# cherubicXN/neat

Hardware: AMD Instinct MI355X
Metric: ray-samples/s (train step) on ABC-neat-a (higher is better)
Workload: dtype bf16; 1 GPU; C2: abc-neat-a networks, 1024 rays x 128 samples per GPU, depth samples given, train step = forward + loss + backward + Adam; rays_per_gpu=1024, samples_per_ray=128, global_rays=1024, parallelism=dp1, weights=synthetic 'rough' (seed 42), launch=hip graph replay, the whole step one launch (forward + loss + backward + Adam)

## Files before the change

neat_amd/csrc/bf16_common.hpp:

```cpp
#pragma once
#include <hip/hip_runtime.h>
#include <stdint.h>

#ifndef NEAT_HALF
#define NEAT_HALF 0
#endif

namespace neat {

struct DevOnce {
  unsigned long long mask = 0;
  static int dev() { int d = 0; if (hipGetDevice(&d) != hipSuccess || d < 0 || d > 63) d = 0; return d; }
  operator bool() const { return ((mask >> dev()) & 1ull) != 0; }
  DevOnce& operator=(bool v) { if (v) mask |= 1ull << dev(); else mask &= ~(1ull << dev()); return *this; }
};
#define NEAT_TRY(expr) do { hipError_t e_ = (expr); if (e_ != hipSuccess) return e_; } while (0)
template <auto... Kerns> hipError_t lds_limit(int bytes) {
  static DevOnce done;
  if (done) return hipSuccess;
  hipError_t e = hipSuccess;
  ((e = e != hipSuccess ? e : hipFuncSetAttribute(reinterpret_cast<const void*>(Kerns), hipFuncAttributeMaxDynamicSharedMemorySize, bytes)), ...);
  if (e == hipSuccess) done = true;
  return e;
}

typedef float f32x16 __attribute__((ext_vector_type(16)));
typedef unsigned short u16;

constexpr int BMH = 128;

typedef float f32x2_t __attribute__((ext_vector_type(2)));
#if NEAT_HALF
typedef _Float16 bf16x8 __attribute__((ext_vector_type(8)));
typedef _Float16 bf16x2_t __attribute__((ext_vector_type(2)));
#define NEAT_MFMA16 __builtin_amdgcn_mfma_f32_32x32x16_f16
__device__ __forceinline__ unsigned pack2(float lo, float hi) {
  f32x2_t v = {lo, hi};
  bf16x2_t r = __builtin_convertvector(v, bf16x2_t);
  return __builtin_bit_cast(unsigned, r);
}
__device__ __forceinline__ u16 f2bf(float f) { return __builtin_bit_cast(u16, (_Float16)f); }
__device__ __forceinline__ float bf2f(u16 h) { return (float)__builtin_bit_cast(_Float16, h); }
__device__ __forceinline__ float bf_lo(unsigned w) { return (float)__builtin_bit_cast(bf16x2_t, w).x; }
__device__ __forceinline__ float bf_hi(unsigned w) { return (float)__builtin_bit_cast(bf16x2_t, w).y; }
#else
typedef __bf16 bf16x8 __attribute__((ext_vector_type(8)));
typedef __bf16 bf16x2_t __attribute__((ext_vector_type(2)));
#define NEAT_MFMA16 __builtin_amdgcn_mfma_f32_32x32x16_bf16
__device__ __forceinline__ unsigned pack2(float lo, float hi) {
  f32x2_t v = {lo, hi};
  bf16x2_t r = __builtin_convertvector(v, bf16x2_t);
  return __builtin_bit_cast(unsigned, r);
}
__device__ __forceinline__ u16 f2bf(float f) { return (u16)(pack2(f, 0.0f) & 0xFFFFu); }
__device__ __forceinline__ float bf2f(u16 h) { return __uint_as_float(((unsigned)h) << 16); }
__device__ __forceinline__ float bf_lo(unsigned w) { return __uint_as_float(w << 16); }
__device__ __forceinline__ float bf_hi(unsigned w) { return __uint_as_float(w & 0xFFFF0000u); }
#endif

typedef short s16x2_t __attribute__((ext_vector_type(2)));
typedef unsigned short u16x2_t __attribute__((ext_vector_type(2)));
__device__ __forceinline__ unsigned pk_relu16(unsigned p) {
  const s16x2_t z = {0, 0};
  return __builtin_bit_cast(unsigned, __builtin_elementwise_max(__builtin_bit_cast(s16x2_t, p), z));
}
__device__ __forceinline__ unsigned pk_nonzero16(unsigned p) {
  unsigned r;
  asm("v_pk_min_u16 %0, %1, %2" : "=v"(r) : "v"(p), "s"(0x00010001u));
  return r;
}
typedef float pk2f_t __attribute__((ext_vector_type(2)));
__device__ __forceinline__ pk2f_t pk_add_f32(pk2f_t a, pk2f_t b) {
  pk2f_t r;
  asm("v_pk_add_f32 %0, %1, %2" : "=v"(r) : "v"(a), "v"(b));
  return r;
}
__device__ __forceinline__ void relu_mask_push(unsigned& m, unsigned relu_pair) { m = (m << 1) | pk_nonzero16(relu_pair); }
__device__ __forceinline__ unsigned relu_mask_word(unsigned m) { return m << 8; }
__device__ __forceinline__ unsigned relu_mask_apply(unsigned& m, unsigned pair) {
  const s16x2_t sh = {15, 15};
  const unsigned keep = __builtin_bit_cast(unsigned, __builtin_bit_cast(s16x2_t, m) >> sh);
  m <<= 1;
  return pair & keep;
}

__device__ __forceinline__ float softplus100_fast(float a) {
  const float u = a * 144.26950408889634f;
  const float y = __builtin_amdgcn_exp2f(-fabsf(u));
  return (fmaxf(u, 0.0f) + __builtin_amdgcn_logf(1.0f + y)) * 0.0069314718055994531f;
}
typedef float v2f_t __attribute__((ext_vector_type(2)));
constexpr float SOFTPLUS_C = 144.26950408889634f;
__device__ __forceinline__ v2f_t softplus100_pk(v2f_t acc, v2f_t bias_scaled) {
  const v2f_t cc = {SOFTPLUS_C, SOFTPLUS_C};
  const v2f_t u = acc * cc + bias_scaled;
  v2f_t y = {__builtin_amdgcn_exp2f(-fabsf(u.x)), __builtin_amdgcn_exp2f(-fabsf(u.y))};
  const v2f_t one = {1.0f, 1.0f};
  y = y + one;
  const v2f_t lg = {__builtin_amdgcn_logf(y.x), __builtin_amdgcn_logf(y.y)};
  const v2f_t m = {fmaxf(u.x, 0.0f), fmaxf(u.y, 0.0f)};
  const v2f_t k = {0.0069314718055994531f, 0.0069314718055994531f};
  return (m + lg) * k;
}
__device__ __forceinline__ float dphi_fast(float h) { return 1.0f - __expf(-100.0f * h); }

struct FusedArgs {
  const float* x_fm; int P, ldp;
  const uint4* Wp[9]; int KS[9]; const float* bias[9];
  int save, values_only;
  u16* h[9];
  float* E;
  u16* feat; float* sdfraw;
  const uint4* Wlo[9]; u16* hlo[9]; u16* featlo;
  float* sdf_out;
  float radius, scale;
  int bias8_rot, bias8_n;
  const int* gate; int gate_value;
};

struct AdjArgs {
  int P, ldp;
  const uint4* Wp[8];
  const u16* h[9];
  u16* u[8];
  const float* w8; const float* rs8;
  float* es; float* e0;
  const uint4* Wlo[8]; const u16* hlo[9];
};

struct HeadX3Args {
  int P, ldp;
  int nvalid;
  const u16* feat; const u16* featlo;
  const float* small; int srows;
  const uint4* Wp[5]; const uint4* Wlo[5];
  const float* bias[5];
  u16* hid[5];
  float* out;
  const u16* smallbf;
  u16* mask[5];
};

struct HeadBwdArgs {
  int P, ldp;
  int nvalid;
  const u16* top;
  const uint4* Wt[5];
  const u16* mask[5];
  u16* ab[4];
  u16* featc;
  int accumulate;
  const float* rho_num; const float* rho_den;
  float* sc; int srows;
};

}
```

neat_amd/csrc/kernels_dw.hpp:

```cpp
#pragma once
#include "kernels_bf16.hpp"

namespace neat {

struct LayerArgsDW {
  LayerArgsWS w;
  const u16* auxA2; int auxA_split;
  int rowsA;
  int P;
  uint4* partial;
  float* pscale;
  float* pbias;
  int ablate;
};

constexpr int DW_MAXSEG = 4;
struct LayerArgsDWSeg { LayerArgsDW l[DW_MAXSEG]; int n; };

constexpr int DW_XLDS = 1024;
constexpr int DW_WG_UINT4 = 8 * 8 * 2 * 64;
#ifndef DW_VALU_PER_MFMA
#define DW_VALU_PER_MFMA 14
#endif

__device__ __forceinline__ unsigned long long dw_uniform64(unsigned long long v) {
  const unsigned lo = __builtin_amdgcn_readfirstlane((unsigned)v), hi = __builtin_amdgcn_readfirstlane((unsigned)(v >> 32));
  return ((unsigned long long)hi << 32) | lo;
}
__device__ __forceinline__ void dw_dma16(unsigned long long sbase, unsigned voff, unsigned lds_dst) {
  unsigned keep;
  asm volatile("s_mov_b32 %0, m0\n\ts_mov_b32 m0, %2\n\ts_nop 0\n\tglobal_load_lds_dwordx4 %1, %3 nt\n\ts_mov_b32 m0, %0"
               : "=&s"(keep) : "v"(voff), "s"(lds_dst), "s"(sbase) : "memory");
}
__device__ __forceinline__ void dw_dma4(unsigned long long sbase, unsigned voff, unsigned lds_dst) {
  unsigned keep;
  asm volatile("s_mov_b32 %0, m0\n\ts_mov_b32 m0, %2\n\ts_nop 0\n\tglobal_load_lds_dword %1, %3\n\ts_mov_b32 m0, %0"
               : "=&s"(keep) : "v"(voff), "s"(lds_dst), "s"(sbase) : "memory");
}

template <int EPI, bool FULL>
__global__ __launch_bounds__(WST, 2) void layer_kernel_wsdw(LayerArgsDWSeg seg) {
  constexpr bool SEG = FULL && EPI != EPI_BWD8;
  typedef WsCfg<EPI, 16> C;
  static_assert(C::NAUX == 2, "tangent / reverse epilogues only");
  constexpr bool TANK = (EPI == EPI_TAN || EPI == EPI_TAN_PF);
  const LayerArgsDW* tab = (const LayerArgsDW*)__builtin_amdgcn_kernarg_segment_ptr();
  const int nlayers = SEG ? seg.n : 1;
  for (int li = 0; li < nlayers; ++li) {
  if (SEG && li > 0) {
    asm volatile("s_waitcnt vmcnt(0)" ::: "memory");
    __syncthreads();
  }
  const LayerArgsDW d = SEG ? tab[li] : seg.l[0];
  const LayerArgsWS& a = d.w;
  extern __shared__ __attribute__((aligned(16))) unsigned char wslds[];
  typedef __attribute__((address_space(3))) void* lds_ptr;
  typedef __attribute__((address_space(3))) v4s16* lds_v4;
  const int lane0 = threadIdx.x & 63;
  const int wave = __builtin_amdgcn_readfirstlane(threadIdx.x >> 6);
  const int t_begin = (int)blockIdx.x, tstride = (int)gridDim.x;
  const int T = (a.ntiles - t_begin + tstride - 1) / tstride;
  const unsigned lds_base = (unsigned)(size_t)(lds_ptr)wslds;
  const unsigned dma_off = (unsigned)(4 * wave) * (WSP * 16);
  constexpr unsigned AUX0 = C::IN_TILE, AUX1 = C::IN_TILE + WS_TILE, EXTRA = C::IN_TILE + WS_TILE * C::NAUX;
  constexpr unsigned AUXA = TANK ? AUX1 : AUX0;
  auto lane_now = [&]() { int l = lane0; asm volatile("" : "+v"(l)); return l; };
  auto dma = [&](const u16* base, int ln, int tile, unsigned dst, int max_oct, const u16* base2, int split) {
    const bool second = 4 * wave >= split;
    const unsigned long long sb = dw_uniform64((unsigned long long)(second ? base2 : base) + (unsigned long long)tile * (WSP * 16));
    const int o0 = second ? 4 * wave - split : 4 * wave;
#pragma unroll
    for (int i = 0; i < 2; ++i) {
      const int opos = 2 * i + (ln >> 5);
      const int oct = min(o0 + opos, second ? 31 : max_oct);
      const unsigned voff = ((unsigned)oct * (unsigned)a.ldp + (unsigned)((ln & 31) ^ (opos << 2))) * 16u;
      dw_dma16(sb, voff, __builtin_amdgcn_readfirstlane(dst + i * (2 * WSP * 16)));
    }
  };
  auto issue = [&](int tau) {
    const unsigned stage = lds_base + (unsigned)(tau % C::NS) * C::STAGE;
    const unsigned slot = stage + dma_off;
    const int tile = t_begin + tau * tstride;
    const int ln = lane_now();
    dma(a.in, ln, tile, slot, a.in_octs - 1, a.in2, a.split_oct);
    dma(a.aux0, ln, tile, slot + AUX0, 31, TANK ? nullptr : d.auxA2, TANK ? (1 << 30) : d.auxA_split);
    dma(a.aux1, ln, tile, slot + AUX1, 31, TANK ? d.auxA2 : nullptr, TANK ? d.auxA_split : (1 << 30));
    if (C::HAS_S) dw_dma4(dw_uniform64((unsigned long long)(a.srow + (size_t)tile * WSP)), (unsigned)(ln & 31) * 4u, __builtin_amdgcn_readfirstlane(stage + EXTRA + wave * 256));
    if (C::HAS_PF) dw_dma16(dw_uniform64((unsigned long long)(a.padfill + (size_t)tile * WSP * 8)), (unsigned)(ln & 31) * 16u, __builtin_amdgcn_readfirstlane(stage + EXTRA));
  };
#pragma unroll
  for (int t = 0; t < C::NS - 1; ++t)
    if (t < T) issue(t);

  const bool live = FULL || wave * 32 < a.N;
  uint4 wreg[16];
#pragma unroll
  for (int ks = 0; ks < 16; ++ks) wreg[ks] = live ? a.Wp[((size_t)wave * a.kstride + ks) * 64 + lane0] : make_uint4(0u, 0u, 0u, 0u);
  float* w8 = reinterpret_cast<float*>(wslds + C::LDS);
  if (EPI == EPI_BWD8 && threadIdx.x < 256) w8[threadIdx.x] = (int)threadIdx.x < a.N ? a.wrow[threadIdx.x] * a.wrow_scale[0] : 0.0f;
  const int Npad = (a.N + 7) & ~7;

  f32x16 dacc[8];
#pragma unroll
  for (int j = 0; j < 8; ++j)
#pragma unroll
    for (int r = 0; r < 16; ++r) dacc[j][r] = 0.0f;
  float bsum[2] = {0.0f, 0.0f};
  const int wr = 64 * (wave >> 1), wc = 128 * (wave & 1);
  const bool BIAS = d.pbias != nullptr && wc == 0;

  for (int tau = 0; tau < T; ++tau) {
    const int ahead = min(C::NS - 2, T - 1 - tau);
    ws_wait_barrier(ahead * C::G);
    if (tau + C::NS - 1 < T) issue(tau + C::NS - 1);
    const unsigned char* slot = wslds + (tau % C::NS) * C::STAGE;
    const int tile = t_begin + tau * tstride;
    const int ln = lane_now();
    const unsigned hi5 = (unsigned)(ln >> 5), l31 = (unsigned)(ln & 31);
    const unsigned G = (unsigned)(ln >> 4), li = (unsigned)(ln & 15);
    const unsigned ol = 2 * (G & 1) + ((li >> 1) & 1);
    const unsigned tro0 = ol * 512 + (((2 * (G >> 1)) ^ ol) * 4 + (li >> 2)) * 16 + (li & 1) * 8;
    const unsigned tro1 = ol * 512 + (((2 * (G >> 1) + 1) ^ ol) * 4 + (li >> 2)) * 16 + (li & 1) * 8;
    const bool tail = (tile + 1) * WSP > d.P;
    const unsigned char* abase = (TANK ? slot + AUX1 : slot) + (wr >> 5) * 2048;
    const unsigned char* bbase = (TANK ? slot : slot + AUX0) + (wc >> 5) * 2048;
    auto frag = [&](const unsigned char* base, int s2) {
      const v4s16 lo = __builtin_amdgcn_ds_read_tr16_b64_v4i16((lds_v4)(base + tro0 + s2 * 256));
      const v4s16 hi = __builtin_amdgcn_ds_read_tr16_b64_v4i16((lds_v4)(base + tro1 + s2 * 256));
      return make_uint4(((const unsigned*)&lo)[0], ((const unsigned*)&lo)[1], ((const unsigned*)&hi)[0], ((const unsigned*)&hi)[1]);
    };
    auto load_frags = [&](int s2, uint4 (&av)[2], uint4 (&bv)[4]) {
#pragma unroll
      for (int i = 0; i < 2; ++i) av[i] = frag(abase + i * 2048, s2);
#pragma unroll
      for (int j = 0; j < 4; ++j) bv[j] = frag(bbase + j * 2048, s2);
    };
    auto mask_frags = [&](int s2, uint4 (&av)[2], uint4 (&bv)[4], bool points) {
      const int arow = wr + (int)(16 * (G & 1) + li);
      const unsigned amask0 = arow < d.rowsA ? 0xFFFFFFFFu : 0u, amask1 = arow + 32 < d.rowsA ? 0xFFFFFFFFu : 0u;
      av[0].x &= amask0; av[0].y &= amask0; av[0].z &= amask0; av[0].w &= amask0;
      av[1].x &= amask1; av[1].y &= amask1; av[1].z &= amask1; av[1].w &= amask1;
      if (!points) return;
      auto mask4 = [&](uint4& v) {
        const int p0 = tile * WSP + 16 * s2 + 8 * (int)(G >> 1);
        unsigned w4[4] = {v.x, v.y, v.z, v.w};
#pragma unroll
        for (int e = 0; e < 4; ++e) {
          const bool k0 = p0 + 2 * e < d.P, k1 = p0 + 2 * e + 1 < d.P;
          w4[e] = (k0 ? (w4[e] & 0x0000FFFFu) : 0u) | (k1 ? (w4[e] & 0xFFFF0000u) : 0u);
        }
        v = make_uint4(w4[0], w4[1], w4[2], w4[3]);
      };
#pragma unroll
      for (int i = 0; i < 2; ++i) mask4(av[i]);
#pragma unroll
      for (int j = 0; j < 4; ++j) mask4(bv[j]);
    };
    auto dw_mma = [&](const uint4 (&av)[2], const uint4 (&bv)[4], bool mfma = true) {
      if (!TANK && BIAS) {
#pragma unroll
        for (int i = 0; i < 2; ++i) {
          const unsigned w4[4] = {av[i].x, av[i].y, av[i].z, av[i].w};
          float t = 0.0f;
#pragma unroll
          for (int e = 0; e < 4; ++e) t += bf_lo(w4[e]) + bf_hi(w4[e]);
          bsum[i] += t;
        }
      }
      if (!mfma) return;
#pragma unroll
      for (int i = 0; i < 2; ++i)
#pragma unroll
        for (int j = 0; j < 4; ++j)
          dacc[i * 4 + j] = NEAT_MFMA16(*reinterpret_cast<const bf16x8*>(&av[i]), *reinterpret_cast<const bf16x8*>(&bv[j]), dacc[i * 4 + j], 0, 0, 0);
    };
    f32x16 acc;
    auto chain = [&]() {
#pragma unroll
      for (int r = 0; r < 16; ++r) acc[r] = 0.0f;
      const unsigned bfrag_e = (hi5 * WSP + (l31 ^ (hi5 << 2))) * 16;
      const unsigned bfrag_o = (hi5 * WSP + (l31 ^ ((2 + hi5) << 2))) * 16;
#pragma unroll
      for (int ks = 0; ks < 16; ++ks) {
        const uint4 bv = *reinterpret_cast<const uint4*>(slot + ((ks & 1) ? bfrag_o : bfrag_e) + ks * (2 * WSP * 16));
        acc = NEAT_MFMA16(*reinterpret_cast<const bf16x8*>(&wreg[ks]), *reinterpret_cast<const bf16x8*>(&bv), acc, 0, 0, 0);
      }
    };
    const int p = tile * WSP + (int)l31;
    auto epi_half = [&](int j, bool fullrows, const uint4* fa = nullptr, const uint4* fb = nullptr) {
      float sp = 0.0f;
      if (C::HAS_S) sp = *reinterpret_cast<const float*>(slot + EXTRA + wave * 256 + l31 * 4);
// ... 195 lines not shown
```

neat_amd/csrc/kernels_heads.hpp:

```cpp
#pragma once
#include "bf16_common.hpp"
#include "fused_launch.hpp"

namespace neat {

struct HC {
  static constexpr int BP = HC_BATCH, THREADS = 512;
  static constexpr int XPL = 32 * BP * 16;
  static constexpr int SPL = 8 * BP * 16;
  static constexpr int XA = 0, XB = XPL, S = 2 * XPL;
  static constexpr int BIAS = S + SPL;
  static constexpr int BIAS_FLOATS = 4 * 256 + 8;
  static constexpr int LDS = BIAS + BIAS_FLOATS * 4;
  static constexpr int KSTEP = 2 * BP * 16;
};

#ifndef NEAT_HC_RING
#define NEAT_HC_RING 3
#endif
#ifndef NEAT_HC_ABLATE
#define NEAT_HC_ABLATE 0
#endif

#ifndef NEAT_HC_NT_FWD
#define NEAT_HC_NT_FWD 1
#endif
#ifndef NEAT_HC_NT_BWD
#define NEAT_HC_NT_BWD 0
#endif
template <bool NT = false>
__device__ __forceinline__ void hc_store8(void* p, uint2 v) {
  typedef unsigned long long u64_t;
  if (NT) __builtin_nontemporal_store(__builtin_bit_cast(u64_t, v), reinterpret_cast<u64_t*>(p));
  else *reinterpret_cast<uint2*>(p) = v;
}
#ifndef NEAT_HC_WIDE
#define NEAT_HC_WIDE 1
#endif
__device__ __forceinline__ uint4 hc_octet(uint2 prev, uint2 cur) {
  typedef unsigned v2u_t __attribute__((ext_vector_type(2)));
  const v2u_t s0 = __builtin_amdgcn_permlane32_swap(prev.x, cur.x, false, false);
  const v2u_t s1 = __builtin_amdgcn_permlane32_swap(prev.y, cur.y, false, false);
  return make_uint4(s0.x, s1.x, s0.y, s1.y);
}
template <bool NT = false>
__device__ __forceinline__ void hc_store16(void* p, uint4 v) {
  typedef unsigned v4u_t __attribute__((ext_vector_type(4)));
  const v4u_t w = {v.x, v.y, v.z, v.w};
  if (NT) __builtin_nontemporal_store(w, reinterpret_cast<v4u_t*>(p));
  else *reinterpret_cast<v4u_t*>(p) = w;
}
#ifndef NEAT_HC_TIMING
#define NEAT_HC_TIMING 0
#endif
#if NEAT_HC_TIMING
#define HC_STAMP(i) do { if (blockIdx.x == 0 && it < 3) { __builtin_amdgcn_s_waitcnt(0); stamp[i] = __builtin_readcyclecounter(); } } while (0)
#else
#define HC_STAMP(i) do { } while (0)
#endif

__device__ __forceinline__ uint4 hc_ldg(const void* base, unsigned off) {
  return *reinterpret_cast<const uint4*>(reinterpret_cast<const unsigned char*>(base) + off);
}
#ifndef NEAT_HC_NT_IN
#define NEAT_HC_NT_IN 0
#endif
__device__ __forceinline__ uint4 hc_ldg_in(const void* base, unsigned off) {
  typedef unsigned v4u_t __attribute__((ext_vector_type(4)));
  if (NEAT_HC_NT_IN) {
    const v4u_t v = __builtin_nontemporal_load(reinterpret_cast<const v4u_t*>(reinterpret_cast<const unsigned char*>(base) + off));
    return make_uint4(v.x, v.y, v.z, v.w);
  }
  return hc_ldg(base, off);
}

template <int KS, bool ZERO, bool ROLL, int NKS, int WN, class Epi>
__device__ __forceinline__ void hc_stage(const unsigned char* fr, uint4 (&w)[WN], f32x16& acc, const void* wn, unsigned woff, Epi&& epi) {
  constexpr int RING = NEAT_HC_RING;
  uint4 b[KS];
#pragma unroll
  for (int i = 0; i < RING && i < KS; ++i) b[i] = *reinterpret_cast<const uint4*>(fr + i * HC::KSTEP);
  if (ROLL) {
#pragma unroll
    for (int ks = KS; ks < NKS; ++ks) w[ks] = hc_ldg(wn, woff + ks * 1024);
  }
  if (ZERO) {
#pragma unroll
    for (int r = 0; r < 16; ++r) acc[r] = 0.0f;
  }
#pragma unroll
  for (int ks = 0; ks < KS; ++ks) {
    if (ks + RING < KS) b[ks + RING] = *reinterpret_cast<const uint4*>(fr + (ks + RING) * HC::KSTEP);
    if (!(NEAT_HC_ABLATE & 2))
      acc = NEAT_MFMA16(*reinterpret_cast<const bf16x8*>(&w[ks]), *reinterpret_cast<const bf16x8*>(&b[ks]), acc, 0, 0, 0);
    else acc[0] += __uint_as_float(w[ks].x ^ b[ks].x);
    if (ROLL && ks < NKS) w[ks] = hc_ldg(wn, woff + ks * 1024);
    if (!(NEAT_HC_ABLATE & 1)) {
#pragma unroll
      for (int e = ks * (16 / KS); e < (ks + 1) * (16 / KS); ++e) epi(e);
    }
    __builtin_amdgcn_sched_barrier(0);
  }
}
template <class Epi> __device__ __forceinline__ void hc_drain(Epi&& epi) {
#pragma unroll
  for (int e = 0; e < 16; ++e) { epi(e); if ((e & 3) == 3) __builtin_amdgcn_sched_barrier(0); }
}

#ifndef NEAT_HC_STAGGER
#define NEAT_HC_STAGGER 0
#endif
struct HcWork {
  int rounds, tail0, grid, nvp;
  __device__ __forceinline__ HcWork(int nvalid_pairs, int g) : grid(g), nvp(nvalid_pairs) {
    rounds = (nvalid_pairs / 2) / g;
    tail0 = rounds * g * 2;
  }
  __device__ __forceinline__ int batch(int it, int bid, int& pair0) const {
    if (NEAT_HC_STAGGER && (bid & 1) && rounds > 0) {
      if (it == 0) { pair0 = 2 * bid; return 1; }
      if (it == rounds) { pair0 = 2 * bid + 1; return 1; }
      if (it > rounds) --it;
    }
    if (it < rounds) { pair0 = 2 * (it * grid + bid); return 2; }
    pair0 = tail0 + (it - rounds) * grid + bid;
    return pair0 < nvp ? 1 : 0;
  }
};

template <int HEAD, bool SAVE>
__global__ __launch_bounds__(512, 2) void head_chain_kernel(HeadX3Args a, int npairs) {
  typedef HC C;
  constexpr int BP = C::BP, NOUT = HEAD ? 6 : 3;
  extern __shared__ __attribute__((aligned(16))) unsigned char hclds[];
  float* biasl = reinterpret_cast<float*>(hclds + C::BIAS);
  const int tid = threadIdx.x, lane = tid & 63, hi = lane >> 5;
  const int wave = __builtin_amdgcn_readfirstlane(tid >> 6);
  for (int idx = tid; idx < 4 * 256; idx += C::THREADS) {
    const int l = idx >> 8, n = idx & 255;
    float v = 0.0f;
#pragma unroll
    for (int k = 0; k < 4; ++k) if (l == k) v = a.bias[k][n];
    biasl[idx] = v;
  }
  if (tid < 8) biasl[4 * 256 + tid] = tid < NOUT ? a.bias[4][tid] : 0.0f;
  for (int idx = tid; idx < C::SPL / 16; idx += C::THREADS) reinterpret_cast<uint4*>(hclds + C::S)[idx] = make_uint4(0u, 0u, 0u, 0u);

  const int nvp = npairs < a.nvalid ? npairs : a.nvalid;
  for (int pair = nvp + blockIdx.x; pair < npairs; pair += gridDim.x) {
    const unsigned p0 = (unsigned)pair * 64u;
    if (SAVE) {
#pragma unroll
      for (int l = 1; l <= 4; ++l) {
#pragma unroll
        for (int i = 0; i < 4; ++i) {
          const int idx = tid + i * C::THREADS, oct = idx >> 6, pp = idx & 63;
          *reinterpret_cast<uint4*>(reinterpret_cast<char*>(a.hid[l]) + ((unsigned)oct * (unsigned)a.ldp + p0 + pp) * 16u) = make_uint4(0u, 0u, 0u, 0u);
        }
        if (tid < 256) reinterpret_cast<uint4*>(reinterpret_cast<char*>(a.mask[l]) + (size_t)pair * 4096)[tid] = make_uint4(0u, 0u, 0u, 0u);
      }
    }
    for (int idx = tid; idx < NOUT * 64; idx += C::THREADS) a.out[(size_t)(idx >> 6) * a.ldp + p0 + (idx & 63)] = 0.0f;
  }

  uint4 w[20], ow[2];
  auto w_off = [&](int KS) -> unsigned {
    unsigned v = (unsigned)((wave * KS) * 64 + lane) * 16u;
    asm volatile("" : "+v"(v));
    return v;
  };
  {
    const unsigned o0 = w_off(20);
#pragma unroll
    for (int ks = 0; ks < 20; ++ks) w[ks] = hc_ldg(a.Wp[0], o0 + ks * 1024);
    unsigned so = (unsigned)(((2 * wave) * 64 + lane) * 16);
    asm volatile("" : "+v"(so));
#pragma unroll
    for (int j = 0; j < 2; ++j) ow[j] = hc_ldg(a.Wp[4], so + j * 1024);
  }
  const unsigned char* frag[3];
  unsigned char* quad[2];
  const unsigned char* biasp;
  {
    const unsigned fo = (unsigned)(hi * BP + (lane & 31)) * 16u, qo = (unsigned)((4 * wave) * BP + (lane & 31)) * 16u + 8u * hi;
    unsigned b0 = C::XA + fo, b1 = C::XB + fo, b2 = C::S + fo, q0 = C::XA + qo, q1 = C::XB + qo, bb = C::BIAS + (unsigned)(32 * wave + 4 * hi) * 4u;
    asm volatile("" : "+v"(b0), "+v"(b1), "+v"(b2), "+v"(q0), "+v"(q1), "+v"(bb));
    frag[0] = hclds + b0; frag[1] = hclds + b1; frag[2] = hclds + b2;
    quad[0] = hclds + q0; quad[1] = hclds + q1; biasp = hclds + bb;
  }
  __syncthreads();

  const HcWork work(nvp, gridDim.x);
  for (int it = 0;; ++it) {
    int pair0;
    const int np = work.batch(it, blockIdx.x, pair0);
    if (np == 0) break;
    const int nt = 2 * np, npts = 64 * np;
#if NEAT_HC_TIMING
    unsigned long long stamp[8];
#endif
    HC_STAMP(0);
    const unsigned p0 = (unsigned)pair0 * 64u;
    unsigned ldp16 = (unsigned)a.ldp * 16u;
    asm volatile("" : "+s"(ldp16));
    const unsigned gquad = ((unsigned)(4 * wave) * (unsigned)a.ldp + p0 + (unsigned)(lane & 31)) * 16u + 8u * hi;
    const unsigned goct = ((unsigned)(4 * wave + hi) * (unsigned)a.ldp + p0 + (unsigned)(lane & 31)) * 16u;
    const unsigned mlane = (((p0 >> 5) * 8u + (unsigned)wave) * 64u + (unsigned)lane) * 4u;
    int tb = tid;
    asm volatile("" : "+v"(tb));
    {
#pragma unroll
      for (int i = 0; i < 8; ++i) {
        const int idx = tb + i * C::THREADS, oct = idx >> 7, pp = idx & 127;
        if (pp < npts) reinterpret_cast<uint4*>(hclds + C::XA)[oct * BP + pp] = hc_ldg_in(a.feat, ((unsigned)oct * (unsigned)a.ldp + p0 + pp) * 16u);
      }
      const int so = tb >> 7, sp = tb & 127;
      for (int o = so; o * 8 < a.srows; o += 4)
        if (sp < npts) reinterpret_cast<uint4*>(hclds + C::S)[o * BP + sp] = hc_ldg_in(a.smallbf, ((unsigned)o * (unsigned)a.ldp + p0 + sp) * 16u);
    }
    __syncthreads();
    HC_STAMP(1);

    f32x16 acc[2];
    unsigned pboff = 0;
    unsigned char* plq = quad[0];
    unsigned pg = 0;
    u16* phout = nullptr; u16* pmout = nullptr; unsigned pmoff = 0;
    float4 bqv = make_float4(0.f, 0.f, 0.f, 0.f);
    unsigned ph[2]; float keep = 0.0f; unsigned mbits = 0;
    uint2 vprev = make_uint2(0u, 0u);
    unsigned pgw = 0;
    auto epi_elem = [&](const f32x16& ap, int e) {
      if (NEAT_HC_ABLATE & 64) {
        keep += ap[e];
        if (e == 15 && keep == 12345.0f) *reinterpret_cast<float*>(plq) = keep;
        return;
      }
      const int q = e >> 2, j = e & 3;
      if (j == 0 && !(NEAT_HC_ABLATE & 32)) bqv = *reinterpret_cast<const float4*>(biasp + pboff + q * 32);
      if ((j & 1) == 0) return;
      const v2f_t av = {ap[e - 1], ap[e]};
      const v2f_t bv = (j == 1) ? v2f_t{bqv.x, bqv.y} : v2f_t{bqv.z, bqv.w};
#ifndef NEAT_HC_PK_BIAS
#define NEAT_HC_PK_BIAS 0
#endif
      const v2f_t rv = NEAT_HC_PK_BIAS ? pk_add_f32(av, bv) : v2f_t{av.x + bv.x, av.y + bv.y};
      const unsigned pr = pk_relu16(pack2(rv.x, rv.y));
      ph[j >> 1] = pr;
      if (SAVE && !(NEAT_HC_ABLATE & 8)) relu_mask_push(mbits, pr);
      if (j != 3) return;
      const uint2 vh = make_uint2(ph[0], ph[1]);
      if (!(NEAT_HC_ABLATE & 16)) *reinterpret_cast<uint2*>(plq + q * (BP * 16)) = vh;
      if (SAVE) {
        if (NEAT_HC_WIDE) {
          if (q & 1) hc_store16<NEAT_HC_NT_FWD != 0>(reinterpret_cast<char*>(phout) + (size_t)(q - 1) * ldp16 + pgw, hc_octet(vprev, vh));
          else vprev = vh;
        } else if (!(NEAT_HC_ABLATE & 4)) hc_store8<NEAT_HC_NT_FWD != 0>(reinterpret_cast<char*>(phout) + (size_t)q * ldp16 + pg, vh);
#ifndef NEAT_HC_NT_MASK
#define NEAT_HC_NT_MASK 1
#endif
        if (q == 3 && !(NEAT_HC_ABLATE & 8)) {
          if (NEAT_HC_NT_MASK) __builtin_nontemporal_store(relu_mask_word(mbits), reinterpret_cast<unsigned*>(reinterpret_cast<char*>(pmout) + pmoff));
          else *reinterpret_cast<unsigned*>(reinterpret_cast<char*>(pmout) + pmoff) = relu_mask_word(mbits);
          mbits = 0;
        }
      }
    };
    auto set_pend = [&](int l, int dst, int t) {
      pboff = (unsigned)l * 1024u;
      plq = quad[dst] + t * 512;
      pg = gquad + (unsigned)t * 512u;
      pgw = goct + (unsigned)t * 512u;
      phout = a.hid[l + 1]; pmout = a.mask[l + 1]; pmoff = mlane + (unsigned)t * 2048u;
    };
    auto none = [](int) {};
    auto seed = [&](f32x16& ac, int t) {
#pragma unroll
      for (int r = 0; r < 16; ++r) ac[r] = 0.0f;
#pragma unroll
      for (int ks = 0; ks < 4; ++ks) {
        const uint4 bs = *reinterpret_cast<const uint4*>(frag[2] + t * 512 + ks * C::KSTEP);
        ac = NEAT_MFMA16(*reinterpret_cast<const bf16x8*>(&w[16 + ks]), *reinterpret_cast<const bf16x8*>(&bs), ac, 0, 0, 0);
      }
    };
#define HC_EPI(ACC_) [&](int e) { epi_elem(ACC_, e); }
#define HC_LAYER(LL, SRC_, DST_, WN_, KSN_)                                                                                        \
    for (int pp = 0; pp < np; ++pp) {                                                                                             \
      const int t0 = 2 * pp;                                                                                                      \
      if (LL == 0) seed(acc[0], t0);                                                                                              \
      if (LL == 0 && pp == 0) {                                                                                                   \
        hc_stage<16, false, false, 16>(frag[SRC_] + t0 * 512, w, acc[0], nullptr, 0u, none);                                       \
      } else {                                                                                                                    \
        if (pp == 0) set_pend(LL - 1, SRC_, nt - 1); else set_pend(LL, DST_, t0 - 1);                                              \
        hc_stage<16, LL != 0, false, 16>(frag[SRC_] + t0 * 512, w, acc[0], nullptr, 0u, HC_EPI(acc[1]));                           \
      }                                                                                                                           \
      if (np == 1 && !(NEAT_HC_ABLATE & 128)) __syncthreads();                                                                    \
      if (LL == 0) seed(acc[1], t0 + 1);                                                                                          \
      set_pend(LL, DST_, t0);                                                                                                     \
      if (pp == np - 1) hc_stage<16, LL != 0, true, 16>(frag[SRC_] + (t0 + 1) * 512, w, acc[1], WN_, w_off(KSN_), HC_EPI(acc[0])); \
      else hc_stage<16, LL != 0, false, 16>(frag[SRC_] + (t0 + 1) * 512, w, acc[1], nullptr, 0u, HC_EPI(acc[0]));                  \
      if (!(NEAT_HC_ABLATE & 128)) __syncthreads();                                                                               \
    }
#define HC_LAYER3 HC_LAYER(3, 1, 0, a.Wp[0], 20)
    HC_LAYER(0, 0, 1, a.Wp[1], 16)
    HC_STAMP(2);
    HC_LAYER(1, 1, 0, a.Wp[2], 16)
    HC_STAMP(3);
    HC_LAYER(2, 0, 1, a.Wp[3], 16)
    HC_STAMP(4);
    HC_LAYER3
    set_pend(3, 0, nt - 1);
    hc_drain(HC_EPI(acc[1]));
    __syncthreads();
    HC_STAMP(5);
#undef HC_LAYER3
#undef HC_LAYER
#undef HC_EPI
    {
      float* red = reinterpret_cast<float*>(hclds + C::XB);
      const unsigned char* fr = frag[0] + (unsigned)(2 * wave) * C::KSTEP;
      for (int t = 0; t < nt; ++t) {
        f32x16 accs;
#pragma unroll
        for (int r = 0; r < 16; ++r) accs[r] = 0.0f;
#pragma unroll
        for (int j = 0; j < 2; ++j) {
          const uint4 bh = *reinterpret_cast<const uint4*>(fr + j * C::KSTEP + t * 512);
          accs = NEAT_MFMA16(*reinterpret_cast<const bf16x8*>(&ow[j]), *reinterpret_cast<const bf16x8*>(&bh), accs, 0, 0, 0);
        }
#pragma unroll
        for (int r = 0; r < 4; ++r) red[(wave * 8 + 4 * hi + r) * BP + t * 32 + (lane & 31)] = accs[r];
      }
      __syncthreads();
      int tf = tid;
      asm volatile("" : "+v"(tf));
      for (int idx = tf; idx < NOUT * BP; idx += C::THREADS) {
        const int n = idx >> 7, pp = idx & 127;
        if (pp < npts) {
          float v = biasl[4 * 256 + n];
#pragma unroll
          for (int wv = 0; wv < 8; ++wv) v += red[(wv * 8 + n) * BP + pp];
          if (HEAD == 0) v = 1.0f / (1.0f + __expf(-v));
          a.out[(size_t)n * a.ldp + p0 + pp] = v;
        }
      }
    }
    __syncthreads();
    HC_STAMP(6);
#if NEAT_HC_TIMING
    if (blockIdx.x == 0 && it < 3 && (tid == 0 || tid == 448))
      printf("hc fwd head %d wave %d batch %d (np %d): load %llu lin0 %llu lin1 %llu lin2 %llu lin3 %llu lin4 %llu cycles\n", HEAD, wave, it, np,
             stamp[1] - stamp[0], stamp[2] - stamp[1], stamp[3] - stamp[2], stamp[4] - stamp[3], stamp[5] - stamp[4], stamp[6] - stamp[5]);
#endif
  }
}


__device__ __forceinline__ float hc_cot_scale_of(const float* slot) {
  if (!slot) return 1.0f;
  const float m = *slot;
  if (!(m > 0.0f) || !(m < 3.0e38f)) return 1.0f;
  int e;
  (void)frexpf(m, &e);
  e = e < -100 ? -100 : (e > 100 ? 100 : e);
  return ldexpf(1.0f, 1 - e);
}

template <int HEAD>
__global__ __launch_bounds__(512, 2) void head_bwd_chain_kernel(HeadBwdArgs a, int npairs) {
  typedef HC C;
  constexpr int BP = C::BP;
  extern __shared__ __attribute__((aligned(16))) unsigned char hclds[];
  const int tid = threadIdx.x, lane = tid & 63, hi = lane >> 5;
  const int wave = __builtin_amdgcn_readfirstlane(tid >> 6);
  for (int idx = tid; idx < C::SPL / 16; idx += C::THREADS) reinterpret_cast<uint4*>(hclds + C::S)[idx] = make_uint4(0u, 0u, 0u, 0u);
  const float rho = a.accumulate ? hc_cot_scale_of(a.rho_num) / hc_cot_scale_of(a.rho_den) : 1.0f;

  const int nvp = npairs < a.nvalid ? npairs : a.nvalid;
  for (int pair = nvp + blockIdx.x; pair < npairs; pair += gridDim.x) {
    const unsigned p0 = (unsigned)pair * 64u;
#pragma unroll
    for (int i = 0; i < 4; ++i) {
      const int idx = tid + i * C::THREADS, oct = idx >> 6, pp = idx & 63;
      const unsigned off = ((unsigned)oct * (unsigned)a.ldp + p0 + pp) * 16u;
#pragma unroll
      for (int l = 0; l < 4; ++l) *reinterpret_cast<uint4*>(reinterpret_cast<char*>(a.ab[l]) + off) = make_uint4(0u, 0u, 0u, 0u);
      if (!a.accumulate) *reinterpret_cast<uint4*>(reinterpret_cast<char*>(a.featc) + off) = make_uint4(0u, 0u, 0u, 0u);
    }
    for (int idx = tid; idx < a.srows * 64; idx += C::THREADS) a.sc[(size_t)(idx >> 6) * a.ldp + p0 + (idx & 63)] = 0.0f;
  }

  uint4 w[16], wtop;
  auto w_off = [&](int tile, int KS) -> unsigned {
    unsigned v = (unsigned)((tile * KS) * 64 + lane) * 16u;
    asm volatile("" : "+v"(v));
    return v;
  };
  wtop = hc_ldg(a.Wt[4], w_off(wave, 4));
  {
    const unsigned o3 = w_off(wave, 16);
#pragma unroll
    for (int ks = 0; ks < 16; ++ks) w[ks] = hc_ldg(a.Wt[3], o3 + ks * 1024);
  }
  const int srt = 8 + (wave >> 2), stile = wave & 3;
  const bool s_live = (srt - 8) * 32 < a.srows;
  const unsigned char* frag[3];
  unsigned char* quad[2];
  {
    const unsigned fo = (unsigned)(hi * BP + (lane & 31)) * 16u, qo = (unsigned)((4 * wave) * BP + (lane & 31)) * 16u + 8u * hi;
    unsigned b0 = C::XA + fo, b1 = C::XB + fo, b2 = C::S + fo, q0 = C::XA + qo, q1 = C::XB + qo;
    asm volatile("" : "+v"(b0), "+v"(b1), "+v"(b2), "+v"(q0), "+v"(q1));
    frag[0] = hclds + b0; frag[1] = hclds + b1; frag[2] = hclds + b2;
    quad[0] = hclds + q0; quad[1] = hclds + q1;
  }
  __syncthreads();

  const HcWork work(nvp, gridDim.x);
  for (int it = 0;; ++it) {
    int pair0;
    const int np = work.batch(it, blockIdx.x, pair0);
    if (np == 0) break;
    const int nt = 2 * np, npts = 64 * np;
    const unsigned p0 = (unsigned)pair0 * 64u;
    unsigned ldp16 = (unsigned)a.ldp * 16u;
    asm volatile("" : "+s"(ldp16));
    const unsigned gquad = ((unsigned)(4 * wave) * (unsigned)a.ldp + p0 + (unsigned)(lane & 31)) * 16u + 8u * hi;
    const unsigned goct = ((unsigned)(4 * wave + hi) * (unsigned)a.ldp + p0 + (unsigned)(lane & 31)) * 16u;
    const unsigned mlane = (((p0 >> 5) * 8u + (unsigned)wave) * 64u + (unsigned)lane) * 4u;
    int tb = tid;
    asm volatile("" : "+v"(tb));
#if NEAT_HC_TIMING
    unsigned long long stamp[8];
#endif
    HC_STAMP(0);
    if (tb < npts) reinterpret_cast<uint4*>(hclds + C::S)[tb] = hc_ldg_in(a.top, (p0 + (unsigned)tb) * 16u);
    __syncthreads();

    f32x16 acc[2];
    unsigned char* plq = quad[0];
    unsigned pg = 0;
    u16* phout = nullptr;
    unsigned pmask = 0, nmask = 0;
    uint2 pf[4], nf[4];
    unsigned ph[2];
    uint2 vprev = make_uint2(0u, 0u);
    unsigned pgw = 0;
    auto ldmask = [&](int l, int t) -> unsigned {
      if (NEAT_HC_NT_MASK) return __builtin_nontemporal_load(reinterpret_cast<const unsigned*>(reinterpret_cast<const char*>(a.mask[l]) + (mlane + (unsigned)t * 2048u)));
      return *reinterpret_cast<const unsigned*>(reinterpret_cast<const char*>(a.mask[l]) + (mlane + (unsigned)t * 2048u));
    };
    auto epi_mask = [&](const f32x16& ap, int e) {
      const int q = e >> 2, j = e & 3;
      if ((j & 1) == 0) return;
      ph[j >> 1] = relu_mask_apply(pmask, pack2(ap[e - 1], ap[e]));
      if (j != 3) return;
      const uint2 vh = make_uint2(ph[0], ph[1]);
      *reinterpret_cast<uint2*>(plq + q * (BP * 16)) = vh;
      if (NEAT_HC_WIDE) {
        if (q & 1) hc_store16<NEAT_HC_NT_BWD != 0>(reinterpret_cast<char*>(phout) + (size_t)(q - 1) * ldp16 + pgw, hc_octet(vprev, vh));
        else vprev = vh;
      } else hc_store8<NEAT_HC_NT_BWD != 0>(reinterpret_cast<char*>(phout) + (size_t)q * ldp16 + pg, vh);
    };
    auto epi_feat = [&](const f32x16& ap, int e) {
      const int q = e >> 2, j = e & 3;
      if ((j & 1) == 0) return;
      v2f_t rv = {ap[e - 1], ap[e]};
      if (HEAD == 1) {
        const unsigned wd = (j & 2) ? pf[q].y : pf[q].x;
        rv = v2f_t{fmaf(rv.x, rho, bf_lo(wd)), fmaf(rv.y, rho, bf_hi(wd))};
      }
      ph[j >> 1] = pack2(rv.x, rv.y);
      if (j != 3) return;
#ifndef NEAT_HC_NT_FEATC
#define NEAT_HC_NT_FEATC 0
#endif
      hc_store8<NEAT_HC_NT_FEATC != 0>(reinterpret_cast<char*>(a.featc) + (size_t)q * ldp16 + pg, make_uint2(ph[0], ph[1]));
    };
    auto set_pend = [&](int l, int dst, int t) {
      plq = quad[dst] + t * 512;
      pg = gquad + (unsigned)t * 512u;
      pgw = goct + (unsigned)t * 512u;
      phout = a.ab[l];
    };
    auto ldfeat = [&](int t) {
      if (HEAD == 1) {
#pragma unroll
        for (int q = 0; q < 4; ++q)
          nf[q] = *reinterpret_cast<const uint2*>(reinterpret_cast<const char*>(a.featc) + (size_t)q * ldp16 + (gquad + (unsigned)t * 512u));
      }
    };
    HC_STAMP(1);
    {
      unsigned m4[4];
#pragma unroll
      for (int t = 0; t < 4; ++t) m4[t] = t < nt ? ldmask(4, t) : 0u;
      auto top_mma = [&](f32x16& ac, int t) {
        const uint4 bs = *reinterpret_cast<const uint4*>(frag[2] + t * 512);
#pragma unroll
        for (int r = 0; r < 16; ++r) ac[r] = 0.0f;
        ac = NEAT_MFMA16(*reinterpret_cast<const bf16x8*>(&wtop), *reinterpret_cast<const bf16x8*>(&bs), ac, 0, 0, 0);
// ... 91 lines not shown
```

neat_amd/csrc/neat_fused.hip:

```cpp
#if defined(NEAT_HALF) && NEAT_HALF
#define neat neat_f16
#endif
#include "kernels_fused.hpp"
#include "kernels_x3.hpp"
#include "kernels_heads.hpp"

namespace neat {

hipError_t launch_sdf_fused_w64(hipStream_t st, const FusedArgs& a, int ntiles, int nwg, bool full) {
  typedef F6Cfg<4, 1> C;
  NEAT_TRY((lds_limit<&sdf_fused_w64_kernel<4, false, 1>, &sdf_fused_w64_kernel<4, true, 1>>(C::LDS)));
  if (full) hipLaunchKernelGGL((sdf_fused_w64_kernel<4, false, 1>), dim3(nwg), dim3(C::THREADS), C::LDS, st, a, ntiles, nwg);
  else hipLaunchKernelGGL((sdf_fused_w64_kernel<4, true, 1>), dim3(nwg), dim3(C::THREADS), C::LDS, st, a, ntiles, nwg);
  return hipGetLastError();
}

hipError_t launch_sdf_adjoint_w64(hipStream_t st, const AdjArgs& a, int ntiles, int nwg, bool save) {
  typedef F6Cfg<4, 1> C;
  NEAT_TRY((lds_limit<&sdf_adjoint_w64_kernel<true>, &sdf_adjoint_w64_kernel<false>>(C::LDS)));
  if (save) hipLaunchKernelGGL((sdf_adjoint_w64_kernel<true>), dim3(nwg), dim3(C::THREADS), C::LDS, st, a, ntiles, nwg);
  else hipLaunchKernelGGL((sdf_adjoint_w64_kernel<false>), dim3(nwg), dim3(C::THREADS), C::LDS, st, a, ntiles, nwg);
  return hipGetLastError();
}

template <auto Kern, class A> static hipError_t x3_launch(hipStream_t st, int nbatches, int nwg, const A& args) {
  NEAT_TRY(lds_limit<Kern>(X3::LDS));
  const int grid = nbatches < nwg ? nbatches : nwg;
  if (grid <= 0) return hipSuccess;
  hipLaunchKernelGGL(Kern, dim3(grid), dim3(X3::THREADS), X3::LDS, st, args, nbatches);
  return hipGetLastError();
}

hipError_t launch_sdf_chain_x3(hipStream_t st, const FusedArgs& a, int nbatches, int nwg, bool full) {
  return full ? x3_launch<&sdf_chain_x3_kernel<false>>(st, nbatches, nwg, a) : x3_launch<&sdf_chain_x3_kernel<true>>(st, nbatches, nwg, a);
}

hipError_t launch_sdf_adjoint_x3(hipStream_t st, const AdjArgs& a, int nbatches, int nwg, bool save) {
  return save ? x3_launch<&sdf_adjoint_x3_kernel<true>>(st, nbatches, nwg, a) : x3_launch<&sdf_adjoint_x3_kernel<false>>(st, nbatches, nwg, a);
}

hipError_t launch_head_chain_x3(hipStream_t st, const HeadX3Args& a, int head, int nbatches, int nwg, bool save) {
  if (head == 0) return save ? x3_launch<&head_chain_x3_kernel<0, true>>(st, nbatches, nwg, a) : x3_launch<&head_chain_x3_kernel<0, false>>(st, nbatches, nwg, a);
  return save ? x3_launch<&head_chain_x3_kernel<1, true>>(st, nbatches, nwg, a) : x3_launch<&head_chain_x3_kernel<1, false>>(st, nbatches, nwg, a);
}

template <auto Kern, class A> static hipError_t hc_launch(hipStream_t st, int npairs, int nwg, const A& args) {
  NEAT_TRY(lds_limit<Kern>(HC::LDS));
  const int nb = (npairs + 1) / 2;
  const int grid = nb < nwg ? nb : nwg;
  if (grid <= 0) return hipSuccess;
  hipLaunchKernelGGL(Kern, dim3(grid), dim3(HC::THREADS), HC::LDS, st, args, npairs);
  return hipGetLastError();
}

hipError_t launch_head_chain(hipStream_t st, const HeadX3Args& a, int head, int npairs, int nwg, bool save) {
  if (head == 0) return save ? hc_launch<&head_chain_kernel<0, true>>(st, npairs, nwg, a) : hc_launch<&head_chain_kernel<0, false>>(st, npairs, nwg, a);
  return save ? hc_launch<&head_chain_kernel<1, true>>(st, npairs, nwg, a) : hc_launch<&head_chain_kernel<1, false>>(st, npairs, nwg, a);
}

hipError_t launch_head_bwd_chain(hipStream_t st, const HeadBwdArgs& a, int head, int npairs, int nwg) {
  return head == 0 ? hc_launch<&head_bwd_chain_kernel<0>>(st, npairs, nwg, a) : hc_launch<&head_bwd_chain_kernel<1>>(st, npairs, nwg, a);
}

}
```

Measured before the change: 50.04 million ray-samples/s.

## Prefetch next batch's head inputs via LDS DMA during last layer

Result: no change. 49.71 million ray-samples/s (-0.7%).

```diff
diff --git a/neat_amd/csrc/bf16_common.hpp b/neat_amd/csrc/bf16_common.hpp
--- a/neat_amd/csrc/bf16_common.hpp
+++ b/neat_amd/csrc/bf16_common.hpp
@@ -26,6 +26,26 @@
 
 typedef float f32x16 __attribute__((ext_vector_type(16)));
 typedef unsigned short u16;
+
+__device__ __forceinline__ unsigned long long dw_uniform64(unsigned long long v) {
+  const unsigned lo = __builtin_amdgcn_readfirstlane((unsigned)v), hi = __builtin_amdgcn_readfirstlane((unsigned)(v >> 32));
+  return ((unsigned long long)hi << 32) | lo;
+}
+template <bool NT = true>
+__device__ __forceinline__ void dw_dma16(unsigned long long sbase, unsigned voff, unsigned lds_dst) {
+  unsigned keep;
+  if (NT)
+    asm volatile("s_mov_b32 %0, m0\n\ts_mov_b32 m0, %2\n\ts_nop 0\n\tglobal_load_lds_dwordx4 %1, %3 nt\n\ts_mov_b32 m0, %0"
+                 : "=&s"(keep) : "v"(voff), "s"(lds_dst), "s"(sbase) : "memory");
+  else
+    asm volatile("s_mov_b32 %0, m0\n\ts_mov_b32 m0, %2\n\ts_nop 0\n\tglobal_load_lds_dwordx4 %1, %3\n\ts_mov_b32 m0, %0"
+                 : "=&s"(keep) : "v"(voff), "s"(lds_dst), "s"(sbase) : "memory");
+}
+__device__ __forceinline__ void dw_dma4(unsigned long long sbase, unsigned voff, unsigned lds_dst) {
+  unsigned keep;
+  asm volatile("s_mov_b32 %0, m0\n\ts_mov_b32 m0, %2\n\ts_nop 0\n\tglobal_load_lds_dword %1, %3\n\ts_mov_b32 m0, %0"
+               : "=&s"(keep) : "v"(voff), "s"(lds_dst), "s"(sbase) : "memory");
+}
 
 constexpr int BMH = 128;
 
diff --git a/neat_amd/csrc/kernels_dw.hpp b/neat_amd/csrc/kernels_dw.hpp
--- a/neat_amd/csrc/kernels_dw.hpp
+++ b/neat_amd/csrc/kernels_dw.hpp
@@ -23,20 +23,6 @@
 #define DW_VALU_PER_MFMA 14
 #endif
 
-__device__ __forceinline__ unsigned long long dw_uniform64(unsigned long long v) {
-  const unsigned lo = __builtin_amdgcn_readfirstlane((unsigned)v), hi = __builtin_amdgcn_readfirstlane((unsigned)(v >> 32));
-  return ((unsigned long long)hi << 32) | lo;
-}
-__device__ __forceinline__ void dw_dma16(unsigned long long sbase, unsigned voff, unsigned lds_dst) {
-  unsigned keep;
-  asm volatile("s_mov_b32 %0, m0\n\ts_mov_b32 m0, %2\n\ts_nop 0\n\tglobal_load_lds_dwordx4 %1, %3 nt\n\ts_mov_b32 m0, %0"
-               : "=&s"(keep) : "v"(voff), "s"(lds_dst), "s"(sbase) : "memory");
-}
-__device__ __forceinline__ void dw_dma4(unsigned long long sbase, unsigned voff, unsigned lds_dst) {
-  unsigned keep;
-  asm volatile("s_mov_b32 %0, m0\n\ts_mov_b32 m0, %2\n\ts_nop 0\n\tglobal_load_lds_dword %1, %3\n\ts_mov_b32 m0, %0"
-               : "=&s"(keep) : "v"(voff), "s"(lds_dst), "s"(sbase) : "memory");
-}
 
 template <int EPI, bool FULL>
 __global__ __launch_bounds__(WST, 2) void layer_kernel_wsdw(LayerArgsDWSeg seg) {
diff --git a/neat_amd/csrc/kernels_heads.hpp b/neat_amd/csrc/kernels_heads.hpp
--- a/neat_amd/csrc/kernels_heads.hpp
+++ b/neat_amd/csrc/kernels_heads.hpp
@@ -13,6 +13,8 @@
   static constexpr int BIAS_FLOATS = 4 * 256 + 8;
   static constexpr int LDS = BIAS + BIAS_FLOATS * 4;
   static constexpr int KSTEP = 2 * BP * 16;
+  static constexpr int RED = BIAS + 4 * 256 * 4;
+  static constexpr int lds_fwd(int nout) { return RED + 8 * nout * 64 * 4; }
 };
 
 #ifndef NEAT_HC_RING
@@ -73,6 +75,10 @@
   }
   return hc_ldg(base, off);
 }
+
+#ifndef NEAT_HC_DMA_IN
+#define NEAT_HC_DMA_IN 1
+#endif
 
 template <int KS, bool ZERO, bool ROLL, int NKS, int WN, class Epi>
 __device__ __forceinline__ void hc_stage(const unsigned char* fr, uint4 (&w)[WN], f32x16& acc, const void* wn, unsigned woff, Epi&& epi) {
@@ -143,7 +149,8 @@
     for (int k = 0; k < 4; ++k) if (l == k) v = a.bias[k][n];
     biasl[idx] = v;
   }
-  if (tid < 8) biasl[4 * 256 + tid] = tid < NOUT ? a.bias[4][tid] : 0.0f;
+  static_assert(NEAT_HC_DMA_IN * NEAT_HC_STAGGER == 0, "the staggered order puts a 2-pair batch behind a single pair: no columns for its second pair");
+  if (!NEAT_HC_DMA_IN && tid < 8) biasl[4 * 256 + tid] = tid < NOUT ? a.bias[4][tid] : 0.0f;
   for (int idx = tid; idx < C::SPL / 16; idx += C::THREADS) reinterpret_cast<uint4*>(hclds + C::S)[idx] = make_uint4(0u, 0u, 0u, 0u);
 
   const int nvp = npairs < a.nvalid ? npairs : a.nvalid;
@@ -191,10 +198,15 @@
   __syncthreads();
 
   const HcWork work(nvp, gridDim.x);
+  typedef __attribute__((address_space(3))) void* lds_ptr;
+  const unsigned lds_base = (unsigned)(size_t)(lds_ptr)hclds;
+  unsigned xnext = C::XB;
+  const float bias4 = __uint_as_float(__builtin_amdgcn_readfirstlane(__float_as_uint(NEAT_HC_DMA_IN && wave < NOUT ? a.bias[4][wave] : 0.0f)));
   for (int it = 0;; ++it) {
-    int pair0;
+    int pair0, pair0n = 0;
     const int np = work.batch(it, blockIdx.x, pair0);
     if (np == 0) break;
+    const int npn = NEAT_HC_DMA_IN ? work.batch(it + 1, blockIdx.x, pair0n) : 0;
     const int nt = 2 * np, npts = 64 * np;
 #if NEAT_HC_TIMING
     unsigned long long stamp[8];
@@ -208,7 +220,7 @@
     const unsigned mlane = (((p0 >> 5) * 8u + (unsigned)wave) * 64u + (unsigned)lane) * 4u;
     int tb = tid;
     asm volatile("" : "+v"(tb));
-    {
+    if (!NEAT_HC_DMA_IN || it == 0) {
 #pragma unroll
       for (int i = 0; i < 8; ++i) {
         const int idx = tb + i * C::THREADS, oct = idx >> 7, pp = idx & 127;
@@ -218,8 +230,22 @@
       for (int o = so; o * 8 < a.srows; o += 4)
         if (sp < npts) reinterpret_cast<uint4*>(hclds + C::S)[o * BP + sp] = hc_ldg_in(a.smallbf, ((unsigned)o * (unsigned)a.ldp + p0 + sp) * 16u);
     }
+    if (NEAT_HC_DMA_IN) asm volatile("s_waitcnt vmcnt(0)" ::: "memory");
     __syncthreads();
     HC_STAMP(1);
+    auto fetch_next = [&](int pp) {
+      unsigned vo = (unsigned)lane * 16u;
+      asm volatile("" : "+v"(vo));
+      constexpr unsigned ROW = BP * 16;
+      const unsigned pt = (unsigned)(pair0n + pp) * 1024u, col = lds_base + (unsigned)pp * 1024u;
+      const unsigned long long fb = dw_uniform64((unsigned long long)a.feat + ((unsigned)(4 * wave) * ldp16 + pt));
+#pragma unroll
+      for (int i = 0; i < 4; ++i)
+        dw_dma16<NEAT_HC_NT_IN != 0>(fb, vo + (unsigned)i * ldp16, __builtin_amdgcn_readfirstlane(col + xnext + (unsigned)(4 * wave + i) * ROW));
+      if (wave * 8 < a.srows)
+        dw_dma16<NEAT_HC_NT_IN != 0>(dw_uniform64((unsigned long long)a.smallbf + ((unsigned)wave * ldp16 + pt)), vo,
+                                     __builtin_amdgcn_readfirstlane(col + (unsigned)C::S + (unsigned)wave * ROW));
+    };
 
     f32x16 acc[2];
     unsigned pboff = 0;
@@ -300,6 +326,7 @@
       if (pp == np - 1) hc_stage<16, LL != 0, true, 16>(frag[SRC_] + (t0 + 1) * 512, w, acc[1], WN_, w_off(KSN_), HC_EPI(acc[0])); \
       else hc_stage<16, LL != 0, false, 16>(frag[SRC_] + (t0 + 1) * 512, w, acc[1], nullptr, 0u, HC_EPI(acc[0]));                  \
       if (!(NEAT_HC_ABLATE & 128)) __syncthreads();                                                                               \
+      if (NEAT_HC_DMA_IN && LL == 3 && pp < npn) fetch_next(pp);                                                                   \
     }
 #define HC_LAYER3 HC_LAYER(3, 1, 0, a.Wp[0], 20)
     HC_LAYER(0, 0, 1, a.Wp[1], 16)
@@ -316,7 +343,38 @@
 #undef HC_LAYER3
 #undef HC_LAYER
 #undef HC_EPI
-    {
+    if (NEAT_HC_DMA_IN) {
+      float* red = reinterpret_cast<float*>(hclds + C::RED);
+      const unsigned char* fr = frag[0] + (unsigned)(2 * wave) * C::KSTEP;
+      for (int pp = 0; pp < np; ++pp) {
+        if (pp) __syncthreads();
+#pragma unroll
+        for (int th = 0; th < 2; ++th) {
+          f32x16 accs;
+#pragma unroll
+          for (int r = 0; r < 16; ++r) accs[r] = 0.0f;
+#pragma unroll
+          for (int j = 0; j < 2; ++j) {
+            const uint4 bh = *reinterpret_cast<const uint4*>(fr + j * C::KSTEP + (2 * pp + th) * 512);
+            accs = NEAT_MFMA16(*reinterpret_cast<const bf16x8*>(&ow[j]), *reinterpret_cast<const bf16x8*>(&bh), accs, 0, 0, 0);
+          }
+#pragma unroll
+          for (int r = 0; r < 4; ++r)
+            if (4 * hi + r < NOUT) red[(wave * NOUT + 4 * hi + r) * 64 + th * 32 + (lane & 31)] = accs[r];
+        }
+        __syncthreads();
+        if (wave < NOUT) {
+          float v = bias4;
+#pragma unroll
+          for (int wv = 0; wv < 8; ++wv) v += red[(wv * NOUT + wave) * 64 + lane];
+          if (HEAD == 0) v = 1.0f / (1.0f + __expf(-v));
+          a.out[(size_t)wave * a.ldp + p0 + pp * 64 + lane] = v;
+        }
+      }
+      const unsigned char* f0 = frag[0]; frag[0] = frag[1]; frag[1] = f0;
+      unsigned char* q0 = quad[0]; quad[0] = quad[1]; quad[1] = q0;
+      xnext ^= (unsigned)(C::XA ^ C::XB);
+    } else {
       float* red = reinterpret_cast<float*>(hclds + C::XB);
       const unsigned char* fr = frag[0] + (unsigned)(2 * wave) * C::KSTEP;
       for (int t = 0; t < nt; ++t) {
@@ -344,8 +402,8 @@
           a.out[(size_t)n * a.ldp + p0 + pp] = v;
         }
       }
-    }
-    __syncthreads();
+      __syncthreads();
+    }
     HC_STAMP(6);
 #if NEAT_HC_TIMING
     if (blockIdx.x == 0 && it < 3 && (tid == 0 || tid == 448))
diff --git a/neat_amd/csrc/neat_fused.hip b/neat_amd/csrc/neat_fused.hip
--- a/neat_amd/csrc/neat_fused.hip
+++ b/neat_amd/csrc/neat_fused.hip
@@ -44,18 +44,19 @@
   return save ? x3_launch<&head_chain_x3_kernel<1, true>>(st, nbatches, nwg, a) : x3_launch<&head_chain_x3_kernel<1, false>>(st, nbatches, nwg, a);
 }
 
-template <auto Kern, class A> static hipError_t hc_launch(hipStream_t st, int npairs, int nwg, const A& args) {
-  NEAT_TRY(lds_limit<Kern>(HC::LDS));
+template <auto Kern, int LDS = HC::LDS, class A> static hipError_t hc_launch(hipStream_t st, int npairs, int nwg, const A& args) {
+  NEAT_TRY(lds_limit<Kern>(LDS));
   const int nb = (npairs + 1) / 2;
   const int grid = nb < nwg ? nb : nwg;
   if (grid <= 0) return hipSuccess;
-  hipLaunchKernelGGL(Kern, dim3(grid), dim3(HC::THREADS), HC::LDS, st, args, npairs);
+  hipLaunchKernelGGL(Kern, dim3(grid), dim3(HC::THREADS), LDS, st, args, npairs);
   return hipGetLastError();
 }
 
 hipError_t launch_head_chain(hipStream_t st, const HeadX3Args& a, int head, int npairs, int nwg, bool save) {
-  if (head == 0) return save ? hc_launch<&head_chain_kernel<0, true>>(st, npairs, nwg, a) : hc_launch<&head_chain_kernel<0, false>>(st, npairs, nwg, a);
-  return save ? hc_launch<&head_chain_kernel<1, true>>(st, npairs, nwg, a) : hc_launch<&head_chain_kernel<1, false>>(st, npairs, nwg, a);
+  constexpr int L0 = NEAT_HC_DMA_IN ? HC::lds_fwd(3) : HC::LDS, L1 = NEAT_HC_DMA_IN ? HC::lds_fwd(6) : HC::LDS;
+  if (head == 0) return save ? hc_launch<&head_chain_kernel<0, true>, L0>(st, npairs, nwg, a) : hc_launch<&head_chain_kernel<0, false>, L0>(st, npairs, nwg, a);
+  return save ? hc_launch<&head_chain_kernel<1, true>, L1>(st, npairs, nwg, a) : hc_launch<&head_chain_kernel<1, false>, L1>(st, npairs, nwg, a);
 }
 
 hipError_t launch_head_bwd_chain(hipStream_t st, const HeadBwdArgs& a, int head, int npairs, int nwg) {
```
